# zkcrypto/bellman

Hardware: AMD Instinct MI355X
Metric: G1 MSM Mscalar-mul/s (BLS12-381, 2^20 bases per GPU) (higher is better)
Workload: dtype u32x12 (381-bit Montgomery integers)

## Files before the change

### bellman_amd/csrc/env_settings.hpp

```cpp
#pragma once
#include <stddef.h>
#include <stdlib.h>

namespace bh {

struct EnvSettings {
  static constexpr size_t UNSET = (size_t)-1;
  int table_max_log2 = -1;
  int table_max_log2_g1 = -1;
  bool table_pad = true;
  bool fft_one_level = true;
  long max_jobs = 0;
  size_t table_budget = UNSET;
  size_t fft_table_budget = UNSET;
  size_t pool_cap = UNSET;
  bool verify_each_shared = false;
  bool debug = false;
};

inline const EnvSettings &env() {
  static const EnvSettings s = [] {
    EnvSettings v;
    auto text = [](const char *name) { const char *e = getenv(name); return e && *e ? e : nullptr; };
    auto log2_limit = [&](const char *name) {
      const char *e = text(name);
      if (!e) return -1;
      const long x = strtol(e, nullptr, 10);
      return (int)(x < 0 ? 0 : x > 24 ? 24 : x);
    };
    auto not_zero = [](const char *name) { const char *e = getenv(name); return !(e && *e == '0'); };
    auto megabytes = [&](const char *name) {
      const char *e = text(name);
      return e ? (size_t)strtoull(e, nullptr, 10) << 20 : EnvSettings::UNSET;
    };
    v.table_max_log2 = log2_limit("BELLMAN_HIP_TABLE_MAX_LOG2");
    v.table_max_log2_g1 = log2_limit("BELLMAN_HIP_TABLE_MAX_LOG2_G1");
    v.table_pad = not_zero("BELLMAN_HIP_TABLE_PAD");
    v.fft_one_level = not_zero("BELLMAN_HIP_FFT_ONE_LEVEL");
    if (const char *e = text("BELLMAN_HIP_MAX_JOBS")) v.max_jobs = strtol(e, nullptr, 10);
    v.table_budget = megabytes("BELLMAN_HIP_TABLE_BUDGET_MB");
    v.fft_table_budget = megabytes("BELLMAN_HIP_FFT_TABLE_BUDGET_MB");
    v.pool_cap = megabytes("BELLMAN_HIP_POOL_CAP_MB");
    if (const char *e = text("BELLMAN_HIP_VERIFY_EACH_SHARED")) v.verify_each_shared = *e != '0';
    v.debug = getenv("BH_DEBUG") != nullptr;
    return v;
  }();
  return s;
}

inline int env_hw_queues() {
  const char *q = getenv("GPU_MAX_HW_QUEUES");
  return (q && *q) ? atoi(q) : 0;
}

}
```

### bellman_amd/csrc/msm_ec.cuh

```cuda
#pragma once
#include <string.h>

#include <algorithm>
#include <type_traits>
#include <vector>
#include <cmath>

#include "fp2pair.cuh"
#include "host_fp.hpp"
#include "msm_scalar.cuh"
#include "msm_types.hpp"

namespace bh {

template <class F>
constexpr u32 default_per_wave() { return F::LANES == 3 ? 21u : F::LANES == 2 ? 32u : 64u; }
template <class F>
constexpr u32 tree_per_wave() { return F::LANES == 3 ? 16u : F::LANES == 2 ? 32u : 64u; }
template <class F>
constexpr u32 workers_per_block(u32 threads, u32 per_wave) { return F::LANES == 1 ? threads : (threads / 64u) * per_wave; }

template <class F>
__device__ __forceinline__ u32 worker_role() {
  if constexpr (F::LANES == 1) return 0u;
// ... 196 lines not shown
  }
  if (blockIdx.x == 0 && density && word_prefix_out)
    for (u32 t = threadIdx.x; t <= nwords; t += blockDim.x) {
      u32 before = 0;
      for (u32 w = 0; w < t && w < nwords; w++) before += (u32)__popcll(density[w]);
      word_prefix_out[t] = before;
    }
  __syncthreads();
  constexpr u32 PW = tree_per_wave<F>();
  const u32 wpb = workers_per_block<F>(SMALL_THREADS, PW);
  const u32 bpb = wpb / SMALL_LANES_PER_BUCKET;
  const u32 bucket_lo = blockIdx.x * bpb;
  for (u32 e = threadIdx.x; e < n_entries; e += blockDim.x) {
    const int d = dig[e];
    if (d == 0) continue;
    const u32 bkt = (u32)(d < 0 ? -d : d) - 1;
    if (bkt < bucket_lo || bkt >= bucket_lo + bpb) continue;
    const u32 slot = atomicAdd(&cnt[bkt - bucket_lo], 1u);
    if (slot < SMALL_LIST_CAP) lists[(bkt - bucket_lo) * SMALL_LIST_CAP + slot] = (unsigned short)e;
  }
  __syncthreads();
  u32 in_block, worker;
  const bool has_worker = worker_index<F>(PW, in_block, worker);
  const u32 nb = 1u << (c - 1);
  const u32 local = in_block / SMALL_LANES_PER_BUCKET, sub = in_block % SMALL_LANES_PER_BUCKET;
  const u32 bkt = bucket_lo + local;
  const bool active = has_worker && local < bpb && bkt < nb;
  const u32 total = active ? cnt[local] : 0;
  XYZZ<F> acc;
  xyzz_set_identity(acc);
  bool saw_identity = false;
  auto add_entry = [&](u32 e) {
    const u32 w = e / nd, i = e - w * nd;
    const u32 k = kidx[i];
    if (k == 0xffffffffu) return;
    Affine<F> q;
    load_affine<F>(q, table + ((u64)w * base_stride + k));
    if (aff_is_identity(q)) { saw_identity = true; return; }
    if (dig[e] < 0) F::neg(q.y, q.y);
    xyzz_madd(acc, q);
  };
  if (total <= SMALL_LIST_CAP) {
    for (u32 t = sub; t < total; t += SMALL_LANES_PER_BUCKET) add_entry(lists[local * SMALL_LIST_CAP + t]);
  } else {
    const int bucket = (int)bkt + 1;
    u32 seen = 0;
    for (u32 e = 0; e < n_entries; e++) {
      const int d = dig[e];
      if (d == bucket || d == -bucket) {
        if (seen % SMALL_LANES_PER_BUCKET == sub) add_entry(e);
        seen++;
      }
    }
  }
  group_reduce_points<F>(acc, SMALL_LANES_PER_BUCKET, sub);
  if (active && sub == 0) store_xyzz<F>(&pts[bkt], acc);
  if (saw_identity) atomicOr(&err->ident, 1u);
}

__device__ __forceinline__ u32 run_last_chunk(const u64 *src, u32 n, u32 z, u32 K, u32 lane, u32 d) {
  const u32 nchunks = (u32)(((u64)(n - z) + K - 1) / K);
  u32 lo = lane + 1, step = 1, hi;
  for (;;) {
    hi = lo + step;
    if (hi >= nchunks) { hi = nchunks; break; }
    if ((u32)(src[(u64)z + (u64)hi * K] >> 32) != d) break;
    lo = hi;
    step <<= 1;
  }
  while (hi - lo > 1) {
    const u32 mid = lo + ((hi - lo) >> 1);
    if ((u32)(src[(u64)z + (u64)mid * K] >> 32) == d) lo = mid; else hi = mid;
  }
  return lo;
}

template <class F>
constexpr int merge_waves_per_simd() { return (F::LANES == 1 && F::WORDS == 24) ? 1 : 2; }
template <class F>
__global__ __launch_bounds__(128, merge_waves_per_simd<F>()) void msm_merge_chunks_kernel(const u64 *pairs, const u32 *zstart,
                                                               XYZZ<typename F::Mem> *pts,
                                                               const XYZZ<typename F::Mem> *head,
                                                               const XYZZ<typename F::Mem> *tail, u32 n, u32 c, u32 K,
                                                               u32 chunks_per_window, u32 walk, LongRun *long_runs,
                                                               u32 max_long, BigRun *big_runs, u32 max_big, u32 big_chunks,
                                                               u32 piece, ErrFlags *err) {
  const u32 w = blockIdx.y;
  u32 in_block, lane;
  if (!worker_index<F>(default_per_wave<F>(), in_block, lane)) return;
  const u64 *src = pairs + (u64)w * n;
  const u32 z = zstart[w];
  K = effective_chunk(n, z, chunks_per_window, K);
  ChunkView v;
  if (lane >= chunks_per_window || !chunk_view(src, n, z, lane, K, v)) return;
  if (!v.tail_partial) return;
  if (v.head_partial && v.d_first == v.d_last) return;
  const u32 d = v.d_last;
  const u32 last = run_last_chunk(src, n, z, K, lane, d);
  if (last - lane > walk) {
    if (worker_role<F>() == 0) {
      if (last - lane > big_chunks) {
        const u32 slot = atomicAdd(&err->nbig, 1u);
        const u32 np = (last - lane + piece) / piece;
        const u32 p0 = atomicAdd(&err->npieces, np);
        if (slot < max_big) { BigRun br = {w, lane, d, last, p0, np, 0u, 0u}; big_runs[slot] = br; }
      } else {
        const u32 slot = atomicAdd(&err->nlong, 1u);
        if (slot < max_long) { LongRun lr = {w, lane, d, last}; long_runs[slot] = lr; }
      }
    }
    return;
  }
  const u64 slot0 = (u64)w * chunks_per_window;
  XYZZ<F> acc;
  load_xyzz<F>(acc, tail + slot0 + lane);
  for (u32 j = lane + 1; j <= last; j++) {
    XYZZ<F> o, r;
    load_xyzz<F>(o, head + slot0 + j);
    xyzz_add(r, acc, o);
    acc = r;
  }
  store_xyzz<F>(&pts[((u64)w << (c - 1)) + d - 1], acc);
}

template <class F>
__device__ __forceinline__ void group_reduce_points(XYZZ<F> &acc, u32 G, u32 sub) {
  constexpr int NW = sizeof(XYZZ<F>) / 4;
  for (u32 off = G >> 1; off >= 1; off >>= 1) {
    XYZZ<F> o;
    u32 *dst = reinterpret_cast<u32 *>(&o);
    const u32 *srcw = reinterpret_cast<const u32 *>(&acc);
#pragma unroll
    for (int i = 0; i < NW; i++) dst[i] = __shfl_down(srcw[i], off * F::LANES);
    if (sub < off) {
      XYZZ<F> r;
      xyzz_add(r, acc, o);
      acc = r;
    }
  }
}

struct HalfPt {
  fp_t u, v;
};
__device__ __forceinline__ fp_t half_sel(bool y, const fp_t &x_v, const fp_t &y_v) {
  fp_t r;
#pragma unroll
  for (int i = 0; i < 12; i++) r.l[i] = y ? y_v.l[i] : x_v.l[i];
  return r;
}
struct PairHalf {
  typedef FpOps F;
  typedef FpOps Mem;
  static constexpr u32 LANES = 2, PER_WAVE = 32;
  __device__ __forceinline__ static bool index(u32 &in_block) { in_block = threadIdx.x >> 1; return true; }
  __device__ __forceinline__ static u32 role() { return k3_lane() & 1u; }
  __device__ __forceinline__ static u32 side() { return role(); }
  __device__ __forceinline__ static fp_t swap(const fp_t &x) {
    fp_t r;
#pragma unroll
    for (int i = 0; i < 12; i++) r.l[i] = (u32)__builtin_amdgcn_update_dpp(0, (int)x.l[i], 0xB1, 0xf, 0xf, false);
    return r;
  }
  __device__ __forceinline__ static bool flag_from(bool mine, u32 want_side) {
    const u32 lane = k3_lane();
    const u64 m = __ballot(mine);
    return (m >> ((lane & ~1u) | want_side)) & 1;
  }
  __device__ __forceinline__ static void load(HalfPt &h, const XYZZ<FpOps> *p) {
    const bool odd = side();
    h.u = odd ? p->y : p->x;
    h.v = odd ? p->zzz : p->zz;
  }
  __device__ __forceinline__ static void store(XYZZ<FpOps> *p, const HalfPt &h) {
    if (side()) { p->y = h.u; p->zzz = h.v; } else { p->x = h.u; p->zz = h.v; }
  }
};
constexpr u32 K6_PER_WAVE = 8;
struct SextetHalf {
  typedef Fp2K3Ops F;
  typedef Fp2Ops Mem;
  static constexpr u32 LANES = 6, PER_WAVE = K6_PER_WAVE;
  __device__ __forceinline__ static bool index(u32 &in_block) {
    const u32 t = (k3_lane() * 43u) >> 8;
    in_block = (threadIdx.x >> 6) * PER_WAVE + t;
    return t < PER_WAVE;
  }
  __device__ __forceinline__ static u32 role() { const u32 l = k3_lane(); return l - 6u * ((l * 43u) >> 8); }
  __device__ __forceinline__ static u32 side() { return role() >= 3u ? 1u : 0u; }
  __device__ __forceinline__ static fp_t swap(const fp_t &x) {
    const int src = (int)k3_lane() + (side() ? -3 : 3);
    fp_t r;
#pragma unroll
    for (int i = 0; i < 12; i++) r.l[i] = (u32)__shfl((int)x.l[i], src);
    return r;
  }
  __device__ __forceinline__ static bool flag_from(bool mine, u32 want_side) {
    const u32 lane = k3_lane();
    const u64 m = __ballot(mine);
    return (m >> (lane - role() + 3u * want_side)) & 1;
  }
  __device__ __forceinline__ static void load(HalfPt &h, const XYZZ<Fp2Ops> *p) {
    const bool y = side();
    Fp2K3Ops::load(h.u, y ? &p->y : &p->x);
    Fp2K3Ops::load(h.v, y ? &p->zzz : &p->zz);
  }
  __device__ __forceinline__ static void store(XYZZ<Fp2Ops> *p, const HalfPt &h) {
    const bool y = side();
    Fp2K3Ops::store(y ? &p->y : &p->x, h.u);
    Fp2K3Ops::store(y ? &p->zzz : &p->zz, h.v);
  }
};
template <class P>
__device__ __forceinline__ bool half_is_identity(const HalfPt &h) { return P::flag_from(P::F::is_zero(h.v), 0u); }
template <class P>
__device__ __forceinline__ void half_add(HalfPt &r, const HalfPt &a, const HalfPt &b) {
  typedef typename P::F F;
  const bool y = P::side();
  if (half_is_identity<P>(a)) { r = b; return; }
  if (half_is_identity<P>(b)) { r = a; return; }
  fp_t t1, t2, d;
  F::mul(t1, a.u, b.v);
  F::mul(t2, b.u, a.v);
  F::sub(d, t2, t1);
  const bool dz = F::is_zero(d);
  if (P::flag_from(dz, 0u)) {
    if (P::flag_from(dz, 1u)) {
      XYZZ<F> full, dbl;
      const fp_t ou = P::swap(a.u), ov = P::swap(a.v);
      full.x = y ? ou : a.u; full.y = y ? a.u : ou;
      full.zz = y ? ov : a.v; full.zzz = y ? a.v : ov;
      xyzz_dbl(dbl, full);
      r.u = y ? dbl.y : dbl.x;
      r.v = y ? dbl.zzz : dbl.zz;
    } else {
      fe_zero(r.u); fe_zero(r.v);
    }
    return;
  }
  fp_t sq, m4, m5, m6, m7;
  F::sqr(sq, d);
  const fp_t osq = P::swap(sq);
  const fp_t pp = y ? osq : sq;
  F::mul(m4, half_sel(y, d, a.v), half_sel(y, sq, b.v));
  const fp_t om4 = P::swap(m4);
  const fp_t ppp = y ? om4 : m4;
  F::mul(m5, t1, half_sel(y, pp, ppp));
  fp_t x3, dq, y3;
  F::sub(x3, osq, ppp);
  F::sub(x3, x3, m5);
  F::sub(x3, x3, m5);
  F::sub(dq, m5, x3);
  const fp_t odq = P::swap(dq);
  F::mul(m6, half_sel(y, a.v, m4), half_sel(y, b.v, ppp));
  F::mul(m7, half_sel(y, m6, d), half_sel(y, pp, odq));
  F::sub(y3, m7, m5);
  r.u = y ? y3 : x3;
  r.v = y ? m6 : m7;
}
template <class P>
__device__ __forceinline__ void half_group_reduce(HalfPt &acc, u32 G, u32 sub) {
  for (u32 off = G >> 1; off >= 1; off >>= 1) {
    HalfPt o;
#pragma unroll
    for (int i = 0; i < 12; i++) {
      o.u.l[i] = __shfl_down(acc.u.l[i], off * P::LANES);
      o.v.l[i] = __shfl_down(acc.v.l[i], off * P::LANES);
    }
    if (sub < off) half_add<P>(acc, acc, o);
  }
}

template <class F>
struct XyzzWorker {
  typedef XYZZ<F> Pt;
  typedef F Ops;
  typedef typename F::Mem Mem;
  static constexpr u32 PER_WAVE = tree_per_wave<F>(), SOLO_PER_WAVE = default_per_wave<F>(), LANES = F::LANES;
  __device__ __forceinline__ static bool index(u32 &in_block, u32 per_wave = PER_WAVE) { u32 g; return worker_index<F>(per_wave, in_block, g); }
  __device__ __forceinline__ static u32 role() { return worker_role<F>(); }
  __device__ __forceinline__ static void identity(Pt &p) { xyzz_set_identity(p); }
  __device__ __forceinline__ static bool is_identity(const Pt &p) { return xyzz_is_identity(p); }
  __device__ __forceinline__ static void load(Pt &p, const XYZZ<Mem> *m) { load_xyzz<F>(p, m); }
  __device__ __forceinline__ static void store(XYZZ<Mem> *m, const Pt &p) { store_xyzz<F>(m, p); }
  __device__ __forceinline__ static void add(Pt &acc, const Pt &o) { Pt r; xyzz_add(r, acc, o); acc = r; }
  __device__ __forceinline__ static void tree(Pt &acc, u32 G, u32 sub) { group_reduce_points<F>(acc, G, sub); }
};
template <class P>
struct HalfWorker {
  typedef HalfPt Pt;
  typedef P Half;
  typedef typename P::Mem Mem;
  static constexpr u32 PER_WAVE = P::PER_WAVE, SOLO_PER_WAVE = P::PER_WAVE, LANES = P::LANES;
  __device__ __forceinline__ static bool index(u32 &in_block, u32 = PER_WAVE) { return P::index(in_block); }
  __device__ __forceinline__ static u32 role() { return P::role(); }
  __device__ __forceinline__ static void identity(Pt &p) { fe_zero(p.u); fe_zero(p.v); }
  __device__ __forceinline__ static bool is_identity(const Pt &p) { return half_is_identity<P>(p); }
  __device__ __forceinline__ static void load(Pt &p, const XYZZ<Mem> *m) { P::load(p, m); }
  __device__ __forceinline__ static void store(XYZZ<Mem> *m, const Pt &p) { P::store(m, p); }
  __device__ __forceinline__ static void add(Pt &acc, const Pt &o) { half_add<P>(acc, acc, o); }
  __device__ __forceinline__ static void tree(Pt &acc, u32 G, u32 sub) { half_group_reduce<P>(acc, G, sub); }
};
typedef HalfWorker<PairHalf> K2Worker;
typedef HalfWorker<SextetHalf> K6Worker;
template <class WK>
__device__ __forceinline__ void fold_over_waves(typename WK::Pt &acc, bool live, u32 PW, u32 wpg, u32 t, typename WK::Pt (*wave_part)[WK::LANES]) {
  const u32 wave = threadIdx.x >> 6, t_in_wave = t - wave * PW, role = WK::role();
  WK::tree(acc, PW, t_in_wave);
  if (live && t_in_wave == 0) wave_part[wave][role] = acc;
  __syncthreads();
  if ((wave & (wpg - 1)) == 0) {
    if (live && t_in_wave < wpg) acc = wave_part[wave + t_in_wave][role]; else WK::identity(acc);
    WK::tree(acc, wpg, t_in_wave);
  }
}

__device__ __forceinline__ u32 nth_with_bit(u32 j, u32 k) { return ((j >> k) << (k + 1)) | (1u << k) | (j & ((1u << k) - 1u)); }
template <class M>
struct SumJob {
  const XYZZ<M> *in;
  XYZZ<M> *out;
  SumDesc d;
  u32 nblocks = 0;
};
template <class M>
struct SumJobs {
  SumJob<M> j[3];
};
template <class WK>
__device__ __forceinline__ void partial_sum(typename WK::Pt &acc, const SumDesc &d, const XYZZ<typename WK::Mem> *in, u32 g, u32 sub, u32 G) {
  const u32 gg = g / d.splits, len = d.count / d.splits, k0 = (g % d.splits) * len;
  const u32 outer = gg / d.inner, in_idx = gg % d.inner;
  const XYZZ<typename WK::Mem> *base = in + ((u64)outer << d.group_shift);
  if (d.mode == SUM_STRIDED) {
    for (u32 k = k0 + sub; k < k0 + len; k += G) {
      typename WK::Pt o;
      WK::load(o, base + (u64)in_idx * d.istride + (u64)k * d.stride);
      WK::add(acc, o);
    }
  } else {
    for (u32 j = sub; j < (d.count >> 1); j += G) {
      typename WK::Pt o;
      WK::load(o, base + nth_with_bit(j, in_idx));
      WK::add(acc, o);
    }
  }
}
template <class WK>
BH_HD constexpr u32 sum_per_wave(u32 lanes) { return (WK::SOLO_PER_WAVE != WK::PER_WAVE && lanes == 1) ? WK::SOLO_PER_WAVE : WK::PER_WAVE; }
template <class F>
constexpr u32 sum_waves() { return F::LANES == 3 ? 4u : 1u; }
template <class WK, u32 NWAVES>
__global__ __launch_bounds__(64 * NWAVES, WK::LANES == 3 ? 2 : 1) void msm_sum_kernel(SumJobs<typename WK::Mem> jobs) {
  typedef typename WK::Pt Pt;
  u32 blk = blockIdx.x;
  u32 which = 0;
  if (blk >= jobs.j[0].nblocks) { blk -= jobs.j[0].nblocks; which = 1; if (blk >= jobs.j[1].nblocks) { blk -= jobs.j[1].nblocks; which = 2; } }
  const SumDesc d = jobs.j[which].d;
  const XYZZ<typename WK::Mem> *in = jobs.j[which].in;
  XYZZ<typename WK::Mem> *out = jobs.j[which].out;
  const u32 PW = sum_per_wave<WK>(d.lanes), WPB = PW * NWAVES;
  u32 t;
  const bool live = WK::index(t, PW);
  const u32 G = d.lanes;
  const u32 g = (blk * WPB + t) / G;
  const u32 sub = t & (G - 1);
  constexpr bool LDS_ACC = (WK::LANES == 1 && sizeof(Pt) > 200);
  __shared__ Pt lds_acc[LDS_ACC ? 64 : 1];
  __shared__ Pt wave_part[NWAVES][WK::LANES];
  Pt reg_acc;
  Pt &acc = LDS_ACC ? lds_acc[threadIdx.x] : reg_acc;
  WK::identity(acc);
  if (live && g < d.groups) partial_sum<WK>(acc, d, in, g, sub, G);
  if constexpr (LDS_ACC) {
    for (u32 off = G >> 1; off >= 1; off >>= 1) {
      __syncthreads();
      if (sub < off) WK::add(lds_acc[threadIdx.x], lds_acc[threadIdx.x + off]);
    }
  } else if (NWAVES == 1 || G <= PW) {
    WK::tree(acc, G, sub);
  } else {
    fold_over_waves<WK>(acc, live, PW, G / PW, t, wave_part);
  }
  if (live && sub == 0 && g < d.groups) WK::store(&out[g], acc);
}
template <class WK, u32 NWAVES>
static u32 sum_count(SumJobs<typename WK::Mem> &js) {
  u32 total = 0;
  for (int q = 0; q < 3; q++) {
    SumJob<typename WK::Mem> &j = js.j[q];
    if (j.d.lanes > NWAVES * WK::PER_WAVE) j.d.lanes = NWAVES * WK::PER_WAVE;
    const u32 wpb = NWAVES * sum_per_wave<WK>(j.d.lanes);
    j.nblocks = (u32)(((u64)j.d.groups * j.d.lanes + wpb - 1) / wpb);
    total += j.nblocks;
  }
  return total;
}
template <class WK, u32 NWAVES>
static bool sum_launch(SumJobs<typename WK::Mem> js, hipStream_t st) {
  const u32 total = sum_count<WK, NWAVES>(js);
  if (!total) return true;
  hipLaunchKernelGGL((msm_sum_kernel<WK, NWAVES>), dim3(total), dim3(64 * NWAVES), 0, st, js);
  return hipGetLastError() == hipSuccess;
}

constexpr u32 LONG_THREADS = 256;
template <class WK>
constexpr u32 long_workers() { return (LONG_THREADS / 64) * WK::PER_WAVE; }
template <class WK>
constexpr u32 long_piece() { return 2 * long_workers<WK>(); }
template <class WK>
__device__ __forceinline__ void long_block_sum(typename WK::Pt &acc, bool live, u32 wid, typename WK::Pt (*wave_part)[WK::LANES]) {
  fold_over_waves<WK>(acc, live, WK::PER_WAVE, LONG_THREADS / 64, wid, wave_part);
  __syncthreads();
}
template <class WK>
__device__ __forceinline__ void merge_medium_runs(XYZZ<typename WK::Mem> *pts, const XYZZ<typename WK::Mem> *head,
                                                  const XYZZ<typename WK::Mem> *tail, u32 c, u32 chunks_per_window,
                                                  const LongRun *runs, u32 nruns, u32 G, u32 wave, u32 nwaves) {
  typedef typename WK::Pt Pt;
  constexpr u32 PW = WK::PER_WAVE;
  u32 wid;
  const bool live = WK::index(wid);
  const u32 t = wid - (threadIdx.x >> 6) * PW;
  const u32 per_wave = PW / G, r = t / G, k = t & (G - 1);
  for (u32 base = wave * per_wave; base < nruns; base += nwaves * per_wave) {
    const u32 e = base + r;
    const bool valid = live && e < nruns;
    LongRun lr = {0, 0, 0, 0};
    if (valid) lr = runs[e];
    const u64 slot0 = (u64)lr.w * chunks_per_window;
    Pt acc;
    WK::identity(acc);
    if (valid) {
      if (k == 0) WK::load(acc, tail + slot0 + lr.lane);
      for (u32 j = lr.lane + 1 + k; j <= lr.last; j += G) {
        Pt o;
        WK::load(o, head + slot0 + j);
        WK::add(acc, o);
      }
    }
    WK::tree(acc, G, k);
    if (valid && k == 0) WK::store(&pts[((u64)lr.w << (c - 1)) + lr.d - 1], acc);
  }
}
template <class WK>
__device__ __forceinline__ void merge_big_runs(XYZZ<typename WK::Mem> *pts, const XYZZ<typename WK::Mem> *head,
                                               const XYZZ<typename WK::Mem> *tail, u32 c, u32 chunks_per_window,
                                               BigRun *runs, u32 nruns, XYZZ<typename WK::Mem> *piece_out, u32 total,
                                               u32 blk, u32 nblk, void *lds_part, u32 *sh_run, u32 *sh_last) {
  typedef typename WK::Pt Pt;
  constexpr u32 NWORK = long_workers<WK>(), PIECE = long_piece<WK>();
  Pt(*wave_part)[WK::LANES] = reinterpret_cast<Pt(*)[WK::LANES]>(lds_part);
  u32 wid;
  const bool live = WK::index(wid);
  for (u32 piece = blk; piece < total; piece += nblk) {
    if (threadIdx.x == 0) *sh_run = 0xffffffffu;
// ... 331 lines not shown
  static_assert(sizeof(typename FR::Mem::T) == sizeof(typename M::T), "both bundles work on the same records");
  typedef XYZZ<M> Pt;
  constexpr bool G2 = (M::WORDS == 24);
  Context &c = *job.ctx;
  hipStream_t st = job.stream;
  const bool use_table = table && !(opts.flags & BH_MSM_NO_TABLE) && (opts.c == 0 || opts.c == table->c) &&
                         (u64)table->W * table->stride < ((u64)1 << 31) && (u64)table->W * n < ((u64)1 << 32);
  if (opts.padded_table && G2) return BH_ERR_INVALID_ARG;
  const MsmPlan p = use_table ? make_table_plan(n, *table, opts.chunk, G2, c.num_cus)
                              : make_plan(n, opts.c, opts.chunk, G2);
  const bool lds_acc = F::LANES == 1 && ((opts.flags & BH_MSM_ACC_LDS) ? true : (opts.flags & BH_MSM_ACC_REGISTERS) ? false : G2);
  job.plan = p;
  if ((u64)p.Wd * n >= ((u64)1 << 32)) return BH_ERR_INVALID_ARG;
  if (n_bases >= ((u64)1 << 31)) return BH_ERR_INVALID_ARG;

  const u64 npairs = (u64)p.Wd * n;
  const u64 ncounts = sort_counts_elems(p);
  const u64 nslots = (u64)p.W * p.chunks_per_window;
  const MergePlan mp = merge_plan<FR>(p, c.num_cus);
  const u32 max_long = mp.max_long, max_big = mp.max_big, max_pieces = mp.max_pieces;
  const u32 H = 1u << p.hi_bits, Lw = 1u << p.lo_bits;
  const u64 nwords = (n + 63) / 64;
  size_t off = 0;
  auto carve = [&](size_t bytes) { const size_t at = off; off += (bytes + 255) & ~size_t(255); return at; };
  const size_t bits_bytes = (size_t)p.W * p.c * sizeof(Pt);
  const size_t o_err = carve(sizeof(ErrFlags));
  const size_t o_bits = carve(bits_bytes);
  const size_t o_pts = carve((u64)p.NB * sizeof(Pt));
  const size_t zero_bytes = off;
  const size_t o_pairs_a = carve(npairs * 8), o_pairs_b = carve(npairs * 8);
  const size_t o_counts = carve((ncounts + 1) * 4), o_scan = carve(scan_tmp_elems(ncounts + 1) * 4), o_zstart = carve((u64)p.W * 4);
  const size_t o_head = carve(nslots * sizeof(Pt)), o_tail = carve(nslots * sizeof(Pt));
  const size_t o_long = carve((u64)max_long * sizeof(LongRun)), o_big = carve((u64)max_big * sizeof(BigRun));
  const size_t o_pieces = carve((u64)max_pieces * sizeof(Pt));
  const size_t o_rowcol = carve((u64)p.W * (H + Lw) * sizeof(Pt));
  constexpr bool TWO_STAGE_FR = std::is_same<FR, FpOps>::value || std::is_same<FR, Fp2K3Ops>::value;
  u32 two_len = 16;
  if (TWO_STAGE_FR) {
    const u64 target = (u64)c.num_cus * 4 * 2 * (G2 ? 16 : 32);
    two_len = 4;
    while (two_len < 64 && 2ull * p.NB / two_len > target) two_len <<= 1;
  }
  const bool want_part = TWO_STAGE_FR && p.NB >= (1u << 17) && p.NB <= (1u << 21) && Lw >= 32 && H >= 32;
  const size_t o_part = want_part ? carve((u64)p.W * ((u64)H * (Lw / std::min(two_len, Lw)) + (u64)Lw * (H / std::min(two_len, H))) * sizeof(Pt)) : 0;
  const size_t o_prefix = density_dev ? carve((nwords + 1) * 4) : 0;
  char *ws = (char *)c.pool.acquire(off);
  if (!ws) return BH_ERR_HIP;
  job.dev_allocs.push_back(ws);
  MsmBuffers b;
  b.err = (ErrFlags *)(ws + o_err);
  b.pairs_a = (u64 *)(ws + o_pairs_a); b.pairs_b = (u64 *)(ws + o_pairs_b);
  b.counts = (u32 *)(ws + o_counts); b.scan_tmp = (u32 *)(ws + o_scan); b.zstart = (u32 *)(ws + o_zstart);
  b.word_prefix = density_dev ? (u32 *)(ws + o_prefix) : nullptr;
  Pt *pts = (Pt *)(ws + o_pts), *head = (Pt *)(ws + o_head), *tail = (Pt *)(ws + o_tail);
  LongRun *long_runs = (LongRun *)(ws + o_long);
  BigRun *big_runs = (BigRun *)(ws + o_big);
  Pt *piece_out = (Pt *)(ws + o_pieces);
  Pt *rowcol = (Pt *)(ws + o_rowcol), *bits = (Pt *)(ws + o_bits);
  Pt *part = want_part ? (Pt *)(ws + o_part) : nullptr;
  ErrFlags *err = b.err;
  job.err_dev = err;
  job.scalars_dev = scalars_dev; job.density_dev = density_dev; job.word_prefix = b.word_prefix;
  const bool from_padded_table = use_table && opts.padded_table;
  job.bases_dev = from_padded_table ? opts.padded_table : bases_dev;
  job.bases_stride = from_padded_table ? 128u : (u32)sizeof(Affine<M>);
  job.skip = skip; job.n_bases = n_bases; job.fmt = fmt;
  job.ref_n = opts.ref_n; job.always_resolve_ident = opts.always_resolve_ident;

  job.timed = (opts.flags & BH_MSM_STAGE_TIMES) != 0;
  if (job.timed) BH_HIP_CHECK(hipEventRecord(job.ev_begin, st));
  BH_HIP_CHECK(hipMemsetAsync(ws, 0, zero_bytes, st));
  const u64 *sorted = nullptr;
  const u32 top_bits = 255u - (p.Wd - 1) * p.c;
  const u64 sliver_load = top_bits >= 31 ? 0 : ((u64)p.nd >> top_bits);
  const bool small_fused = use_table && !opts.padded_table && p.W == 1 && p.nd <= SMALL_MAX_SCALARS && p.n <= SMALL_MAX_ENTRIES &&
                           (u64)p.n <= (u64)SMALL_MAX_PER_BUCKET * p.nb && p.c <= 15 && small_fill_lds_bytes(p.nd, p.n) <= 64 * 1024 &&
                           sliver_load + (u64)p.n / p.nb <= SMALL_LIST_CAP / 2 && !(opts.flags & BH_MSM_NO_SMALL_PATH);
  if (small_fused) {
    const u32 bpb = workers_per_block<F>(SMALL_THREADS, tree_per_wave<F>()) / SMALL_LANES_PER_BUCKET;
    const size_t lds = small_fill_lds_bytes(p.nd, p.n);
    hipLaunchKernelGGL(msm_small_fill_kernel<F>, dim3((p.nb + bpb - 1) / bpb), dim3(SMALL_THREADS), lds, st, scalars_dev, fmt, p.nd,
                       density_dev, b.word_prefix, (u64)skip, (u64)n_bases, p.c, p.Wd, p.base_stride,
                       (const Affine<M> *)bases_dev, pts, err);
    BH_HIP_CHECK(hipGetLastError());
  } else {
    int rc = msm_run_stages(p, b, scalars_dev, fmt, density_dev, skip, n_bases, st, &sorted);
    if (rc) return rc;
  }
  if (job.timed) BH_HIP_CHECK(hipEventRecord(job.ev_sorted, st));
  const bool hold = (opts.flags & BH_MSM_HOLD) != 0;
  if (hold) {
    if (!job.res.sort_event) BH_HIP_CHECK(hipEventCreateWithFlags(&job.res.sort_event, hipEventDisableTiming));
    BH_HIP_CHECK(hipEventRecord(job.res.sort_event, st));
    std::lock_guard<std::mutex> g(c.acc_mu);
    if (c.pending_barriers.size() < 32) c.pending_barriers.push_back(job.res.sort_event);
  }
  Context *cp = &c;
  MsmJobImpl *jp = &job;
  job.resume = [=]() -> int {
  Context &c = *cp;
  MsmJobImpl &job = *jp;
  if (small_fused) {
    if (job.timed) BH_HIP_CHECK(hipEventRecord(job.ev_accum, st));
  } else {
    const dim3 grid = accumulate_grid<F>(p);
    const Affine<M> *bases = (const Affine<M> *)bases_dev;
    const bool padded = opts.padded_bases && !use_table && !G2 && F::LANES == 1 && !lds_acc;
    const bool padded_tab = opts.padded_table && use_table;
    const bool chained = (u64)grid.x * grid.y * 128 >= (u64)c.num_cus * 4 * 64;
    std::unique_lock<std::mutex> chain_lock(c.acc_mu, std::defer_lock);
    if (chained) {
      if (!job.res.acc_event) BH_HIP_CHECK(hipEventCreateWithFlags(&job.res.acc_event, hipEventDisableTiming));
      chain_lock.lock();
      if (c.last_acc_event) BH_HIP_CHECK(hipStreamWaitEvent(st, c.last_acc_event, 0));
      for (hipEvent_t ev : c.pending_barriers) BH_HIP_CHECK(hipStreamWaitEvent(st, ev, 0));
      c.pending_barriers.clear();
    }
    const Affine<M> *acc_bases = padded_tab ? (const Affine<M> *)opts.padded_table : padded ? (const Affine<M> *)opts.padded_bases : bases;
    const u32 acc_stride = (padded || padded_tab) ? 128u : (u32)sizeof(Affine<M>);
    if (int rc = launch_accumulate<F>(st, p, lds_acc, sorted, b.zstart, acc_bases, acc_stride, pts, head, tail, err)) return rc;
    if (chained) {
      BH_HIP_CHECK(hipEventRecord(job.res.acc_event, st));
      c.last_acc_event = job.res.acc_event;
      chain_lock.unlock();
    }
    if (job.timed) BH_HIP_CHECK(hipEventRecord(job.ev_accum, st));
    if (int rc = launch_merges<FR>(st, p, mp, c.num_cus, 0, sorted, b.zstart, pts, head, tail, long_runs, big_runs, piece_out, err)) return rc;
  }
  Pt *rows = rowcol, *cols = rowcol + (u64)p.W * H;
  typedef XyzzWorker<FR> FullWK;
  constexpr u32 NW = sum_waves<FR>(), PW = NW * FullWK::PER_WAVE;
  auto pick_lanes = [&](u32 groups, u32 count) {
    const double slots = (double)c.num_cus * 4;
    u32 best = 1;
    double best_cost = 1e30;
    for (u32 g = 1, lg = 0; g <= PW; g <<= 1, lg++) {
      if (g > count && g > 1) break;
      const double steps = (double)((count + g - 1) / g) + lg + ((FR::LANES == 3 && g > 16) ? 2.0 : 0.0);
      const double waves = (double)groups * g / (double)PW * (double)NW;
      const double cost = steps * std::max(1.0, waves / slots);
      if (cost < best_cost) { best_cost = cost; best = g; }
    }
    return best;
  };
  auto make_job = [&](const Pt *in, Pt *out, SumDesc d) {
    SumJob<M> j;
    d.lanes = d.groups ? pick_lanes(d.groups, d.mode == SUM_BITS ? std::max(1u, d.count / 2) : d.count) : 1;
    j.in = in; j.out = out; j.d = d;
    return j;
  };
  auto launch_sums = [&](SumJobs<M> js, int force = 0) -> bool {
    if constexpr (std::is_same<FR, FpOps>::value) {
      constexpr double K2_SUM_FILL = 4.0;
      u32 groups_all = 0, max_sel = 0;
      for (int q = 0; q < 3; q++)
        if (js.j[q].d.groups) {
          groups_all += js.j[q].d.groups;
          max_sel = std::max(max_sel, js.j[q].d.mode == SUM_BITS ? js.j[q].d.count / 2 : js.j[q].d.count / js.j[q].d.splits);
        }
      if (force == 0 && max_sel >= 128 && groups_all <= 2u * (u32)c.num_cus) {
        const bool four = 2 * 64 < max_sel;
        for (int q = 0; q < 3; q++) js.j[q].d.lanes = (four ? 4 : 2) * K2Worker::PER_WAVE;
        return four ? sum_launch<K2Worker, 4>(js, st) : sum_launch<K2Worker, 2>(js, st);
      }
      if (force != 2 && (force == 1 || (double)sum_count<FullWK, NW>(js) * 2 <= K2_SUM_FILL * (double)c.num_cus * 4))
        return sum_launch<K2Worker, 1>(js, st);
    }
    if constexpr (std::is_same<FR, Fp2K3Ops>::value) {
      constexpr double K6_SUM_FILL = 8.0;
      SumJobs<M> k6 = js;
      if (force != 2 && (double)sum_count<K6Worker, 4>(k6) <= K6_SUM_FILL * (double)c.num_cus) return sum_launch<K6Worker, 4>(k6, st);
    }
    return sum_launch<FullWK, NW>(js, st);
  };
  {
    const u32 cb = p.c - 1;
    SumDesc dr, dc;
    dr.mode = SUM_STRIDED; dr.groups = p.W * H; dr.count = Lw; dr.inner = H; dr.stride = 1; dr.istride = Lw; dr.group_shift = cb;
    dc = dr; dc.groups = p.W * Lw; dc.count = H; dc.inner = Lw; dc.stride = Lw; dc.istride = 1;
    SumJobs<M> js;
    js.j[0] = make_job(pts, rows, dr); js.j[1] = make_job(pts, cols, dc); js.j[2] = js.j[1]; js.j[2].d.groups = 0;
    if (part) {
      const bool one_lane = G2;
      const u32 len_r = std::min(two_len, Lw), len_c = std::min(two_len, H);
      const u32 Sr = Lw / len_r, Sc = H / len_c;
      Pt *part_r = part, *part_c = part + (u64)dr.groups * Sr;
      SumDesc r1 = dr, c1 = dc;
      r1.splits = Sr; r1.groups = dr.groups * Sr; r1.lanes = 1;
      c1.splits = Sc; c1.groups = dc.groups * Sc; c1.lanes = 1;
      SumJobs<M> s1;
      s1.j[0].in = pts; s1.j[0].out = Sr > 1 ? part_r : rows; s1.j[0].d = r1;
      s1.j[1].in = pts; s1.j[1].out = Sc > 1 ? part_c : cols; s1.j[1].d = c1;
      s1.j[2] = s1.j[1]; s1.j[2].d.groups = 0;
      if (!launch_sums(s1, one_lane ? 2 : 1)) return BH_ERR_HIP;
      SumDesc r2, c2;
      r2.mode = SUM_STRIDED; r2.groups = dr.groups; r2.count = Sr; r2.inner = dr.groups; r2.stride = 1; r2.istride = Sr; r2.group_shift = 0;
      c2 = r2; c2.groups = dc.groups; c2.count = Sc; c2.inner = dc.groups; c2.istride = Sc;
      SumJobs<M> s2;
      s2.j[0] = make_job(part_r, rows, r2); if (Sr <= 1) s2.j[0].d.groups = 0;
      s2.j[1] = make_job(part_c, cols, c2); if (Sc <= 1) s2.j[1].d.groups = 0;
      s2.j[2] = s2.j[1]; s2.j[2].d.groups = 0;
      if (!launch_sums(s2, 1)) return BH_ERR_HIP;
      js.j[0].d.groups = js.j[1].d.groups = 0;
    }
    if (G2 && FR::LANES == 1) {
      const double simds = (double)c.num_cus * 4;
      double best = 1e30;
      u32 best_r = js.j[0].d.lanes, best_c = js.j[1].d.lanes;
      for (u32 gr = 1, lr = 0; gr <= 64 && gr <= std::max(1u, dr.count); gr <<= 1, lr++)
        for (u32 gc = 1, lc = 0; gc <= 64 && gc <= std::max(1u, dc.count); gc <<= 1, lc++) {
          const double steps = std::max((double)((dr.count + gr - 1) / gr) + lr, (double)((dc.count + gc - 1) / gc) + lc);
          const double waves = ((double)dr.groups * gr + (double)dc.groups * gc) / 64.0;
          const double cost = steps * std::max(1.0, waves / simds);
          if (cost < best) { best = cost; best_r = gr; best_c = gc; }
        }
      js.j[0].d.lanes = best_r;
      js.j[1].d.lanes = best_c;
    }
    if (!launch_sums(js)) return BH_ERR_HIP;
    SumDesc bl, bh_, bt;
    bl.mode = SUM_BITS; bl.stride = 1; bl.istride = 0;
    bl.groups = p.W * p.lo_bits; bl.count = Lw; bl.inner = std::max(1u, p.lo_bits); bl.group_shift = p.lo_bits;
    bh_ = bl; bh_.groups = p.W * p.hi_bits; bh_.count = H; bh_.inner = std::max(1u, p.hi_bits); bh_.group_shift = p.hi_bits;
    const bool t_from_cols = Lw < H;
    bt.mode = SUM_STRIDED; bt.groups = p.W; bt.count = t_from_cols ? Lw : H; bt.inner = 1; bt.stride = 1; bt.istride = 0;
    bt.group_shift = t_from_cols ? p.lo_bits : p.hi_bits;
    js.j[0] = make_job(cols, bits, bl);
    js.j[1] = make_job(rows, bits + (u64)p.W * p.lo_bits, bh_);
    js.j[2] = make_job(t_from_cols ? cols : rows, bits + (u64)p.W * cb, bt);
    if (!launch_sums(js)) return BH_ERR_HIP;
  }
  if (job.timed) BH_HIP_CHECK(hipEventRecord(job.ev_end, st));
  job.host_result_bytes = (o_bits - o_err) + bits_bytes;
  if (job.host_result_bytes > job.res.pinned_bytes) return BH_ERR_INVALID_ARG;
  BH_HIP_CHECK(hipMemcpyAsync(job.host_result, ws + o_err, job.host_result_bytes, hipMemcpyDeviceToHost, st));
  return BH_OK;
  };
  if (hold) return BH_OK;
  const int rc2 = job.resume();
  job.resume = nullptr;
  return rc2;
}

template <> struct HostOf<FpOps> { typedef HostFpOps type; };
template <> struct HostOf<Fp2Ops> { typedef HostFp2Ops type; };

template <class F>
static void msm_host_tail(const MsmPlan &p, const XYZZ<F> *bits_dev_layout, void *out_dev_layout) {
  typedef typename HostOf<F>::type H;
  static_assert(sizeof(XYZZ<H>) == sizeof(XYZZ<F>) && sizeof(Affine<H>) == sizeof(Affine<F>), "layout");
  std::vector<XYZZ<F>> canon(bits_dev_layout, bits_dev_layout + (size_t)p.W * p.c);
  for (XYZZ<F> &q : canon) { F::canon(q.x); F::canon(q.y); F::canon(q.zz); F::canon(q.zzz); }
  const XYZZ<H> *bits = reinterpret_cast<const XYZZ<H> *>(canon.data());
  XYZZ<H> acc;
  xyzz_set_identity(acc);
  const u32 cb = p.c - 1;
  const XYZZ<H> *lo = bits, *hi = bits + (size_t)p.W * p.lo_bits, *tot = bits + (size_t)p.W * cb;
  for (int w = (int)p.W - 1; w >= 0; w--) {
    for (int b = (int)p.c - 1; b >= 0; b--) {
      XYZZ<H> t;
      xyzz_dbl(t, acc);
      acc = t;
      if (b < (int)cb) {
        const XYZZ<H> &u = (b >= (int)p.lo_bits) ? hi[(size_t)w * p.hi_bits + (b - p.lo_bits)]
                                                 : lo[(size_t)w * p.lo_bits + b];
        xyzz_add(t, acc, u);
        acc = t;
      }
      if (b == 0) {
        xyzz_add(t, acc, tot[w]);
        acc = t;
      }
    }
  }
  Affine<H> res;
  xyzz_to_affine(res, acc);
  memcpy(out_dev_layout, &res, sizeof res);
}

template <class F>
static int msm_finish(MsmJobImpl &job, void *out_affine, float *ms) {
  Context &c = *job.ctx;
  int rc = BH_OK;
  if (job.trivial) {
    memset(out_affine, 0, sizeof(Affine<F>));
    if (ms) ms[0] = ms[1] = ms[2] = ms[3] = 0.f;
    return job.early_rc;
  }
  if (job.resume) {
    rc = job.resume();
    job.resume = nullptr;
  }
  if (hipStreamSynchronize(job.stream) != hipSuccess) rc = BH_ERR_HIP;
  if (rc == BH_OK) {
    const MsmPlan &p = job.plan;
    constexpr size_t ERR_SLOT = 256;
    ErrFlags ef;
    memcpy(&ef, job.host_result, sizeof ef);
    if (ms) {
      ms[0] = ms[1] = ms[2] = ms[3] = 0.f;
      if (job.timed) {
        (void)hipEventElapsedTime(&ms[0], job.ev_begin, job.ev_end);
        (void)hipEventElapsedTime(&ms[1], job.ev_begin, job.ev_sorted);
        (void)hipEventElapsedTime(&ms[2], job.ev_sorted, job.ev_accum);
        (void)hipEventElapsedTime(&ms[3], job.ev_accum, job.ev_end);
      }
    }
    job.saw_eof = ef.eof != 0;
    job.saw_ident = ef.ident != 0;
    job.done_stats[0] = (u64)p.W * p.n; job.done_stats[1] = ef.zeros; job.done_stats[2] = ef.madds;
    job.done_stats[3] = (u64)p.W * p.chunks_per_window; job.done_stats[4] = p.c; job.done_stats[5] = p.chunk;
    job.done_stats[6] = p.W; job.done_stats[7] = p.Wd;
    if (ef.ident && (ef.eof || job.always_resolve_ident)) {
      const u64 nref = job.ref_n ? job.ref_n : p.nd;
      const double c_ln = (nref < 32) ? 3.0 : std::ceil(std::log((double)nref));
      const u32 c_ref = (u32)c_ln, w_ref = (255 + c_ref - 1) / c_ref, lo_ref = c_ref * (w_ref - 1);
      hipLaunchKernelGGL(msm_err_resolve_kernel<F>, dim3((p.nd + 255) / 256), dim3(256), 0, job.stream,
                         job.scalars_dev, job.fmt, p.nd, job.density_dev, job.word_prefix, job.skip, job.n_bases,
                         (const Affine<F> *)job.bases_dev, job.bases_stride, lo_ref, job.err_dev);
      if (hipMemcpyAsync(&ef, job.err_dev, sizeof ef, hipMemcpyDeviceToHost, job.stream) != hipSuccess ||
          hipStreamSynchronize(job.stream) != hipSuccess)
        rc = BH_ERR_HIP;
      else {
        job.saw_ident_top = ef.ident_top != 0;
        rc = !ef.eof ? BH_ERR_UNEXPECTED_IDENTITY : ef.ident_top ? BH_ERR_UNEXPECTED_IDENTITY : BH_ERR_UNEXPECTED_EOF;
      }
    } else if (ef.eof) {
      rc = BH_ERR_UNEXPECTED_EOF;
    } else if (ef.ident) {
      rc = BH_ERR_UNEXPECTED_IDENTITY;
    } else {
      msm_host_tail<F>(p, (const XYZZ<F> *)((const char *)job.host_result + ERR_SLOT), out_affine);
    }
  }
  for (void *ptr : job.dev_allocs) c.pool.release(ptr);
  job.dev_allocs.clear();
  return rc;
}


template <class F>
static int fixed_base_mul_t(const void *base_host, const void *scalars_dev, u64 n, int fmt, void *out_dev,
                            hipStream_t st, void *table_dev) {
  const u32 blocks = (u32)((n + 127) / 128);
  if (!blocks) return BH_OK;
  Affine<F> b;
  memcpy(&b, base_host, sizeof b);
  Affine<F> *table = (Affine<F> *)table_dev;
  hipLaunchKernelGGL(fixed_base_rows_kernel<F>, dim3(1), dim3(64), 0, st, b, table);
  BH_HIP_CHECK(hipGetLastError());
  hipLaunchKernelGGL(fixed_base_table_kernel<F>, dim3((FB_ROWS * FB_COLS + 127) / 128), dim3(128), 0, st, table);
  BH_HIP_CHECK(hipGetLastError());
  hipLaunchKernelGGL(fixed_base_mul_kernel<F>, dim3(blocks), dim3(128), 0, st, (const Affine<F> *)table, scalars_dev, fmt, n,
                     (Affine<F> *)out_dev);
  BH_HIP_CHECK(hipGetLastError());
// ... 176 lines not shown
```

Baseline: 349.2.

## Add four-lane-per-point XYZZ addition worker for bucket-sum reductions

Introduces a QuadHalf worker that spreads each XYZZ point across four lanes, one coordinate per lane, and implements point addition with DPP lane permutes. It is used by default in place of the two-lane K2 worker for the high-fill sum launches and the second-stage partial sums. The aim is more parallelism per point in the small, latency-bound reduction kernels. The cost is more cross-lane permutes and some wasted lanes in the select and doubling paths. An environment variable can turn it off.

```diff
diff --git a/bellman_amd/csrc/env_settings.hpp b/bellman_amd/csrc/env_settings.hpp
--- a/bellman_amd/csrc/env_settings.hpp
+++ b/bellman_amd/csrc/env_settings.hpp
@@ -14,6 +14,7 @@
   size_t table_budget = UNSET;
   size_t fft_table_budget = UNSET;
   size_t pool_cap = UNSET;
+  bool sum_quads = true;
   bool verify_each_shared = false;
   bool debug = false;
 };
@@ -37,6 +38,7 @@
     v.table_max_log2_g1 = log2_limit("BELLMAN_HIP_TABLE_MAX_LOG2_G1");
     v.table_pad = not_zero("BELLMAN_HIP_TABLE_PAD");
     v.fft_one_level = not_zero("BELLMAN_HIP_FFT_ONE_LEVEL");
+    v.sum_quads = not_zero("BELLMAN_HIP_SUM_QUADS");
     if (const char *e = text("BELLMAN_HIP_MAX_JOBS")) v.max_jobs = strtol(e, nullptr, 10);
     v.table_budget = megabytes("BELLMAN_HIP_TABLE_BUDGET_MB");
     v.fft_table_budget = megabytes("BELLMAN_HIP_FFT_TABLE_BUDGET_MB");
diff --git a/bellman_amd/csrc/msm_ec.cuh b/bellman_amd/csrc/msm_ec.cuh
--- a/bellman_amd/csrc/msm_ec.cuh
+++ b/bellman_amd/csrc/msm_ec.cuh
@@ -372,6 +372,7 @@
 struct PairHalf {
   typedef FpOps F;
   typedef FpOps Mem;
+  typedef HalfPt Pt;
   static constexpr u32 LANES = 2, PER_WAVE = 32;
   __device__ __forceinline__ static bool index(u32 &in_block) { in_block = threadIdx.x >> 1; return true; }
   __device__ __forceinline__ static u32 role() { return k3_lane() & 1u; }
@@ -400,6 +401,7 @@
 struct SextetHalf {
   typedef Fp2K3Ops F;
   typedef Fp2Ops Mem;
+  typedef HalfPt Pt;
   static constexpr u32 LANES = 6, PER_WAVE = K6_PER_WAVE;
   __device__ __forceinline__ static bool index(u32 &in_block) {
     const u32 t = (k3_lane() * 43u) >> 8;
@@ -491,6 +493,102 @@
   }
 }
 
+struct QuadPt {
+  fp_t c;
+};
+static_assert(sizeof(XYZZ<FpOps>) == 4 * sizeof(fp_t), "QuadHalf::load / store index the record's coordinates");
+struct QuadHalf {
+  typedef FpOps F;
+  typedef FpOps Mem;
+  typedef QuadPt Pt;
+  static constexpr u32 LANES = 4, PER_WAVE = 16;
+  static constexpr int SWAP2 = 0x4E, LANE0 = 0x00, LANE1 = 0x55, LANE2 = 0xAA, LANE3 = 0xFF;
+  __device__ __forceinline__ static bool index(u32 &in_block) { in_block = threadIdx.x >> 2; return true; }
+  __device__ __forceinline__ static u32 role() { return k3_lane() & 3u; }
+  __device__ __forceinline__ static u32 side() { return role(); }
+  template <int CTRL>
+  __device__ __forceinline__ static fp_t perm(const fp_t &x) {
+    fp_t r;
+#pragma unroll
+    for (int i = 0; i < 12; i++) r.l[i] = (u32)__builtin_amdgcn_update_dpp(0, (int)x.l[i], CTRL, 0xf, 0xf, false);
+    return r;
+  }
+  __device__ __forceinline__ static bool flag_from(bool mine, u32 want_role) {
+    const u32 lane = k3_lane();
+    const u64 m = __ballot(mine);
+    return (m >> ((lane & ~3u) | want_role)) & 1;
+  }
+  __device__ __forceinline__ static void load(QuadPt &h, const XYZZ<FpOps> *p) {
+    h.c = (&p->x)[role()];
+  }
+  __device__ __forceinline__ static void store(XYZZ<FpOps> *p, const QuadPt &h) {
+    (&p->x)[role()] = h.c;
+  }
+};
+__device__ __forceinline__ fp_t quad_sel(u32 role, const fp_t &v0, const fp_t &v1, const fp_t &v2, const fp_t &v3) {
+  fp_t r;
+#pragma unroll
+  for (int i = 0; i < 12; i++) r.l[i] = role == 0 ? v0.l[i] : role == 1 ? v1.l[i] : role == 2 ? v2.l[i] : v3.l[i];
+  return r;
+}
+__device__ __forceinline__ bool quad_is_identity(const QuadPt &h) { return QuadHalf::flag_from(FpOps::is_zero(h.c), 2u); }
+__device__ __forceinline__ void quad_add(QuadPt &r, const QuadPt &a, const QuadPt &b) {
+  typedef FpOps F;
+  typedef QuadHalf Q4;
+  const u32 role = Q4::role();
+  if (quad_is_identity(a)) { r = b; return; }
+  if (quad_is_identity(b)) { r = a; return; }
+  fp_t m1, m2, m3, m4, d;
+  F::mul(m1, a.c, Q4::perm<Q4::SWAP2>(b.c));
+  F::sub(d, Q4::perm<Q4::SWAP2>(m1), m1);
+  const bool dz = F::is_zero(d);
+  if (Q4::flag_from(dz, 0u)) {
+    if (Q4::flag_from(dz, 1u)) {
+      XYZZ<F> full, dbl;
+      full.x = Q4::perm<Q4::LANE0>(a.c); full.y = Q4::perm<Q4::LANE1>(a.c);
+      full.zz = Q4::perm<Q4::LANE2>(a.c); full.zzz = Q4::perm<Q4::LANE3>(a.c);
+      xyzz_dbl(dbl, full);
+      const u32 k0 = 0u - (u32)(role == 0), k1 = 0u - (u32)(role == 1), k2 = 0u - (u32)(role == 2), k3 = 0u - (u32)(role == 3);
+#pragma unroll
+      for (int i = 0; i < 12; i++) r.c.l[i] = (dbl.x.l[i] & k0) | (dbl.y.l[i] & k1) | (dbl.zz.l[i] & k2) | (dbl.zzz.l[i] & k3);
+    } else {
+      fe_zero(r.c);
+    }
+    return;
+  }
+  const bool lo = role < 2u;
+  F::mul(m2, half_sel(lo, a.c, d), half_sel(lo, b.c, d));
+  const fp_t pp = Q4::perm<Q4::LANE0>(m2), p0 = Q4::perm<Q4::LANE0>(d);
+  F::mul(m3, quad_sel(role, m1, p0, m2, m2), pp);
+  const fp_t ppp = Q4::perm<Q4::LANE1>(m3), q = Q4::perm<Q4::LANE0>(m3), rr = Q4::perm<Q4::LANE1>(m2);
+  const fp_t s1 = Q4::perm<Q4::LANE1>(m1);
+  fp_t x3, dq, y3;
+  F::sub(x3, rr, ppp);
+  F::sub(x3, x3, q);
+  F::sub(x3, x3, q);
+  F::sub(dq, q, x3);
+  const bool y = role == 1u;
+  F::mul(m4, quad_sel(role, s1, d, m2, m2), half_sel(y, ppp, dq));
+  F::sub(y3, m4, Q4::perm<Q4::LANE0>(m4));
+  r.c = quad_sel(role, x3, y3, m3, m4);
+}
+__device__ __forceinline__ void half_group_reduce_quads(QuadPt &acc, u32 G, u32 sub) {
+  for (u32 off = G >> 1; off >= 1; off >>= 1) {
+    QuadPt o;
+#pragma unroll
+    for (int i = 0; i < 12; i++) o.c.l[i] = __shfl_down(acc.c.l[i], off * QuadHalf::LANES);
+    if (sub < off) quad_add(acc, acc, o);
+  }
+}
+__device__ __forceinline__ void lane_pt_zero(HalfPt &p) { fe_zero(p.u); fe_zero(p.v); }
+__device__ __forceinline__ void lane_pt_zero(QuadPt &p) { fe_zero(p.c); }
+template <class P> __device__ __forceinline__ bool lane_pt_is_identity(const HalfPt &p) { return half_is_identity<P>(p); }
+template <class P> __device__ __forceinline__ bool lane_pt_is_identity(const QuadPt &p) { return quad_is_identity(p); }
+template <class P> __device__ __forceinline__ void lane_pt_add(HalfPt &acc, const HalfPt &o) { half_add<P>(acc, acc, o); }
+template <class P> __device__ __forceinline__ void lane_pt_add(QuadPt &acc, const QuadPt &o) { quad_add(acc, acc, o); }
+template <class P> __device__ __forceinline__ void lane_pt_tree(HalfPt &acc, u32 G, u32 sub) { half_group_reduce<P>(acc, G, sub); }
+template <class P> __device__ __forceinline__ void lane_pt_tree(QuadPt &acc, u32 G, u32 sub) { half_group_reduce_quads(acc, G, sub); }
+
 template <class F>
 struct XyzzWorker {
   typedef XYZZ<F> Pt;
@@ -508,21 +606,22 @@
 };
 template <class P>
 struct HalfWorker {
-  typedef HalfPt Pt;
+  typedef typename P::Pt Pt;
   typedef P Half;
   typedef typename P::Mem Mem;
   static constexpr u32 PER_WAVE = P::PER_WAVE, SOLO_PER_WAVE = P::PER_WAVE, LANES = P::LANES;
   __device__ __forceinline__ static bool index(u32 &in_block, u32 = PER_WAVE) { return P::index(in_block); }
   __device__ __forceinline__ static u32 role() { return P::role(); }
-  __device__ __forceinline__ static void identity(Pt &p) { fe_zero(p.u); fe_zero(p.v); }
-  __device__ __forceinline__ static bool is_identity(const Pt &p) { return half_is_identity<P>(p); }
+  __device__ __forceinline__ static void identity(Pt &p) { lane_pt_zero(p); }
+  __device__ __forceinline__ static bool is_identity(const Pt &p) { return lane_pt_is_identity<P>(p); }
   __device__ __forceinline__ static void load(Pt &p, const XYZZ<Mem> *m) { P::load(p, m); }
   __device__ __forceinline__ static void store(XYZZ<Mem> *m, const Pt &p) { P::store(m, p); }
-  __device__ __forceinline__ static void add(Pt &acc, const Pt &o) { half_add<P>(acc, acc, o); }
-  __device__ __forceinline__ static void tree(Pt &acc, u32 G, u32 sub) { half_group_reduce<P>(acc, G, sub); }
+  __device__ __forceinline__ static void add(Pt &acc, const Pt &o) { lane_pt_add<P>(acc, o); }
+  __device__ __forceinline__ static void tree(Pt &acc, u32 G, u32 sub) { lane_pt_tree<P>(acc, G, sub); }
 };
 typedef HalfWorker<PairHalf> K2Worker;
 typedef HalfWorker<SextetHalf> K6Worker;
+typedef HalfWorker<QuadHalf> K4Worker;
 template <class WK>
 __device__ __forceinline__ void fold_over_waves(typename WK::Pt &acc, bool live, u32 PW, u32 wpg, u32 t, typename WK::Pt (*wave_part)[WK::LANES]) {
   const u32 wave = threadIdx.x >> 6, t_in_wave = t - wave * PW, role = WK::role();
@@ -1160,6 +1259,11 @@
   auto launch_sums = [&](SumJobs<M> js, int force = 0) -> bool {
     if constexpr (std::is_same<FR, FpOps>::value) {
       constexpr double K2_SUM_FILL = 4.0;
+      const bool quads = env().sum_quads;
+      if (force == 3) {
+        if (quads) return sum_launch<K4Worker, 2>(js, st);
+        force = 1;
+      }
       u32 groups_all = 0, max_sel = 0;
       for (int q = 0; q < 3; q++)
         if (js.j[q].d.groups) {
@@ -1169,6 +1273,7 @@
       if (force == 0 && max_sel >= 128 && groups_all <= 2u * (u32)c.num_cus) {
         const bool four = 2 * 64 < max_sel;
         for (int q = 0; q < 3; q++) js.j[q].d.lanes = (four ? 4 : 2) * K2Worker::PER_WAVE;
+        if (quads) return four ? sum_launch<K4Worker, 8>(js, st) : sum_launch<K4Worker, 4>(js, st);
         return four ? sum_launch<K2Worker, 4>(js, st) : sum_launch<K2Worker, 2>(js, st);
       }
       if (force != 2 && (force == 1 || (double)sum_count<FullWK, NW>(js) * 2 <= K2_SUM_FILL * (double)c.num_cus * 4))
@@ -1208,7 +1313,7 @@
       s2.j[0] = make_job(part_r, rows, r2); if (Sr <= 1) s2.j[0].d.groups = 0;
       s2.j[1] = make_job(part_c, cols, c2); if (Sc <= 1) s2.j[1].d.groups = 0;
       s2.j[2] = s2.j[1]; s2.j[2].d.groups = 0;
-      if (!launch_sums(s2, 1)) return BH_ERR_HIP;
+      if (!launch_sums(s2, 3)) return BH_ERR_HIP;
       js.j[0].d.groups = js.j[1].d.groups = 0;
     }
     if (G2 && FR::LANES == 1) {
```

After: 346.1. No clear change (-0.9%).
